# tungphambasement/DCNN

Hardware: AMD Instinct MI355X
Metric: images/sec (whole node) ResNet-18 Tiny-ImageNet training at 1/2/4/8 MI355X (higher is better)
Workload: dtype bf16; 1 GPU; model=resnet18_tiny_imagenet, global_batch=256, per_gpu_batch=256, parallelism=dp1, optimizer=adam, hipgraph=True, engine=native (C++ host API)

## Files before the change

### dcnn_amd/csrc/kernels/api.h

```cpp
#pragma once
#include <hip/hip_runtime.h>
#include <stdint.h>

#include "fusion_plan.h"
typedef __bf16 bf16;

namespace dcnn {
struct BnbArgs {
  const bf16* y; const bf16* x; const float* mean; const float* istd;
  const float* gamma; const float* beta; int mask_x;
};
struct NtArgs {
  const bf16* A; const bf16* B; void* C;
  int M, N, K; int lda, ldb, ldc; int mode;
  int nb, sh, sw, cs, gh, gw; int kh, kw, strh, strw, padh, padw;
  const float* bias; const bf16* residual; float* stats; int out_f32; int relu;
};
struct TnArgs {
  const bf16* dY; const bf16* X; float* slab; float* bias_slab;
  int M, N, P; int mode; int nb, sh, sw, cs, gh, gw; int kh, kw, strh, strw, padh, padw; int ldx; int k_per_split;
};
struct G2Args {
  const bf16* A; const bf16* B; bf16* C;
  unsigned a_bytes, b_bytes;
// ... 38 lines not shown
  int NB, H, W, Cs, N, ldb, ntaps;
  int tap_dy[9], tap_dx[9], tap_b[9];
  int TH, TW, IMG, HPR;
  const float* bias; const bf16* residual; float* stats; int relu;
  float* zero_ptr; int zero_n;
  BnbArgs bnb;
  float* Cf; const float* residual_f;
  int splits; float* part; unsigned* tickets;
};
void hconv(HConvArgs a, hipStream_t s);
int hconv_splits(int NB, int H, int W, int Cs, int N, int ntaps);
int hconv_tiles(int NB, int H, int W, int Cs, int N, int ntaps);
int hconv_tile_elems(int NB, int H, int W, int Cs, int N, int ntaps);
int hconv_split_target();
void gemm_t2_set_split_target(int t);
void hwgrad_set_split_target(int t);
void hconv3_set_max_splits(int n);
void g1s_set_waves_per_simd(int w);
void hconv_set_split_target(int t);
void hconv_set_split_min_work(int w);
void bn_set_vectorised(int on);
bool hconv_supported(int NB, int H, int W, int Cs, int N, int ntaps);
int hconv_stat_rows(int NB, int H, int W, int Cs, int N, int ntaps, int f32out);
bool hconv3_f32_try(const HConvArgs& a, hipStream_t s);
int hconv3_f32_splits(int NB, int H, int W, int Cs, int N, int ntaps);
bool hconv_v3(int NB, int H, int W, int Cs, int N, int ntaps);
void hconv3_enable(int on);
void hconv3_set_grid_cap(int n);
void hconv3_set_stamps(uintptr_t p);
struct HWArgs {
  const bf16* dY; const bf16* X; float* slab; float* bias_slab;
  unsigned dy_bytes, x_bytes;
  int NB, H, W, Cs, Co, ntaps;
  int tap_dy[9], tap_dx[9];
  int TH, TW, IMG, HPR, tiles_per_split;
  int ldy, ldx, npairs;
  int pair_yoff[3], pair_xoff[3], pair_bias[3];
};
void hwgrad(HWArgs a, int splits, hipStream_t s);
bool hwgrad_supported(int NB, int H, int W, int Cs, int Co, int ntaps);
int hwgrad_splits(int NB, int H, int W, int Cs, int Co);
bool hwgrad_f32_supported(int NB, int H, int W, int Cs, int Co);
int hwgrad_f32_splits(int NB, int H, int W, int Cs, int Co);
void hwgrad_f32(HWArgs a, int splits, hipStream_t s);
void hwgrad_set_version(int v);
bool hwgrad_s2_supported(int NB, int H, int W, int Cs, int Co);
int hwgrad_s2_splits(int NB, int H, int W, int Cs, int Co);
void hwgrad_s2(HWArgs a, int splits, hipStream_t s);

void gemm_nt(const NtArgs& a, hipStream_t s);
void gemm_g2(const G2Args& a, hipStream_t s);
void gemm_g2_set_splitk(int on);
int gemm_g2_splitk_enabled();
int gemm_g2_stat_rows(int M, int N);
int gemm_g2_row_tile(int M, int N);
void gemm_t2(T2Args a, int splits, hipStream_t s);
int g1s_rows(int M, int N, int K, int mode);
void g1s_enable(int on);
void g1s(const bf16* X, const bf16* Wt, bf16* Y, int M, int N, int K, int H, int W, int OH, int OW, int S,
         const float* bias, const bf16* residual, float* stats, int relu, float* zero_ptr, int zero_n, BnbArgs bnb,
         int mode, hipStream_t s);
int g1s_gen_rows(int M, int N, int Kc, int ntaps, int mode);
void g1s_gen(const bf16* X, const bf16* Wt, bf16* Y, int NB, int GH, int GW, int N, int Kc, int ldw,
             const std::vector<std::array<int, 3>>& taps, int H, int W, int OHo, int OWo, int OS, int ORY, int ORX,
             const bf16* residual, float* stats, float* zero_ptr, int zero_n, BnbArgs bnb, int mode, hipStream_t s);
int gemm_t2_splits(int M, int N, int P);
int gemm_nt_stat_rows(int M, int N);
void elementwise(int mode, int op, const float* a, const float* b, float* c, long n, float s0, float s1, hipStream_t s);
void reduce(int op, const float* a, const float* b, long n, float* workspace, float* out, hipStream_t s);
void fill_random(float* out, long n, uint64_t seed, float a, float b, int normal, hipStream_t s);
void transpose_batched(const float* in, float* out, int batch, int rows, int cols, hipStream_t s);
void transpose_batched16(const void* in, void* out, int batch, int rows, int cols, hipStream_t s);
void rows_copy(int kind, const void* src, int lds, void* dst, int ldd, long rows, int cols, hipStream_t s);
void nchw_cnhw(const float* in, float* out, int N, int C, int HW, int to_cnhw, hipStream_t s);
void pad_crop(const float* in, float* out, int NC, int H, int W, int OH, int OW, int top, int left, float value,
              hipStream_t s);
void gemm_g2f(const G2Args& a, hipStream_t s);
int gemm_g2f_stat_rows(int M, int N);
void gemm_t2f(T2Args a, int splits, hipStream_t s);
int gemm_t2f_splits(int M, int N, int P);
void set_f32_mode(int mode);
int get_f32_mode();
void conv_weight_transpose_f32(const float* w, float* wt, int Co, int T_, int Ci, hipStream_t s);
void gemm_tn(TnArgs a, int splits, hipStream_t s);
int gemm_tn_splits(int M, int N, int P);
int gemm_tn_k_per_split(int P, int splits);
int gemm_tn_bias_rows(int M);
struct ConvRouteGeom {
  int N, C, H, W, Co, KH, KW, SH, SW, PH, PW, OH, OW, g1s_mode;
};
enum ConvRoute : int { ROUTE_GENERIC = 0, ROUTE_GEMM_G2 = 1, ROUTE_HALO = 2, ROUTE_G1S = 3, ROUTE_HALO_S2 = 4 };
int conv_fwd_route(ConvRouteGeom g);
int conv_dgrad_route(ConvRouteGeom g);
int conv_wgrad_route(ConvRouteGeom g);
void splitk_reduce(const float* slab, float* out, long n, int splits, int accumulate, hipStream_t s);
void splitk_reduce2(const float* slab, float* out, long n, const float* bslab, float* bout, long nb, int splits,
                    int accumulate, hipStream_t s);

constexpr int kMaxRed = 48;
struct RedEnt { const float* slab; float* out; long n; int splits, unit0, chunks, groups, vec, wpc; };
struct MultiRed { int count; RedEnt e[kMaxRed]; };
void multi_splitk_reduce(MultiRed t, hipStream_t s);

int bn_partial_rows(long R, int C);
void bn_partial(int dtype, const void* x, const void* dy, const void* yout, void* dy_out, const float* mean,
                const float* istd, long R, int C, float* slab, int mode, float* zero_sums, hipStream_t s);
// ... 143 lines not shown
```

### dcnn_amd/csrc/kernels/bindings.cpp

```cpp
#include <tuple>
#include <pybind11/pybind11.h>
#include <pybind11/stl.h>
#include <algorithm>
#include <array>
#include <vector>
#include <hip/hip_runtime.h>
#include <stdint.h>

namespace py = pybind11;
#include "api.h"


using namespace dcnn;
void bind_runtime(py::module_& m);
void bind_rccl(py::module_& m);
template <typename T>
static inline T P(uintptr_t x) { return reinterpret_cast<T>(x); }
static inline hipStream_t S(uintptr_t x) { return reinterpret_cast<hipStream_t>(x); }

using Ptr4 = std::array<uintptr_t, 4>;
static BnbArgs bnb_of(const Ptr4& b) {
  return BnbArgs{P<const bf16*>(b[0]), P<const bf16*>(b[1]), P<const float*>(b[2]), P<const float*>(b[3])};
}

// ... 102 lines not shown
  m.def("hconv_stat_rows", &hconv_stat_rows);
  m.def("hconv_splits", &hconv_splits);
  m.def("hconv_tiles", &hconv_tiles);
  m.def("hconv_set_split_target", &hconv_set_split_target);
  m.def("hconv_set_split_min_work", &hconv_set_split_min_work);
  m.def("hconv_split_target", &hconv_split_target);
  m.def("gemm_t2_set_split_target", &gemm_t2_set_split_target);
  m.def("hwgrad_set_split_target", &hwgrad_set_split_target);
  m.def("hconv3_set_max_splits", &hconv3_set_max_splits);
  m.def("bn_set_vectorised", &bn_set_vectorised);
  m.def("hconv_tile_elems", &hconv_tile_elems);
  m.def("hconv3_set_grid_cap", &hconv3_set_grid_cap);
  m.def("hconv3_enable", &hconv3_enable);
  m.def("hconv_v3", &hconv_v3);
  m.def("hconv3_set_stamps", &hconv3_set_stamps);
  m.def("hwgrad",
        [](int kind, uintptr_t dY, uintptr_t X, uintptr_t slab, uintptr_t bias_slab, unsigned dy_bytes,
           unsigned x_bytes, int NB, int H, int W, int Cs, int Co, const WgradTaps& taps, int splits, int ldy, int ldx,
           const std::vector<std::array<int, 3>>& pairs, uintptr_t stream) {
          HWArgs a{};
          if (pairs.size() > 3) throw std::runtime_error("hwgrad: at most 3 operand pairs");
          a.npairs = (int)pairs.size(); a.ldy = ldy; a.ldx = ldx;
          for (size_t q = 0; q < pairs.size(); ++q) {
            a.pair_yoff[q] = pairs[q][0]; a.pair_xoff[q] = pairs[q][1]; a.pair_bias[q] = pairs[q][2];
          }
          a.dY = P<const bf16*>(dY); a.X = P<const bf16*>(X); a.slab = P<float*>(slab);
          a.bias_slab = P<float*>(bias_slab);
          a.dy_bytes = dy_bytes; a.x_bytes = x_bytes;
          a.NB = NB; a.H = H; a.W = W; a.Cs = Cs; a.Co = Co;
          if (kind == 1) {
            a.ntaps = 9;
            hwgrad_s2(a, splits, S(stream));
            return;
          }
          set_taps(a, taps, "hwgrad");
          if (kind == 2)
            hwgrad_f32(a, splits, S(stream));
          else
            hwgrad(a, splits, S(stream));
        });
  m.def("hwgrad_supported", &hwgrad_supported);
  m.def("hwgrad_s2_supported", &hwgrad_s2_supported);
  m.def("hwgrad_s2_splits", &hwgrad_s2_splits);
  m.def("hwgrad_f32_supported", &hwgrad_f32_supported);
  m.def("hwgrad_f32_splits", &hwgrad_f32_splits);
  m.def("split3_bf16", [](uintptr_t in, uintptr_t out, long rows, int C, int pattern, uintptr_t st) {
    split3_bf16(P<const float*>(in), P<bf16*>(out), rows, C, pattern, S(st));
  });
  m.def("hwgrad_splits", &hwgrad_splits);
  m.def("hwgrad_set_version", &hwgrad_set_version);
  m.def("gemm_g2f_stat_rows", &gemm_g2f_stat_rows);
  m.def("gemm_g2_set_splitk", &gemm_g2_set_splitk);
  m.def("gemm_g2_splitk_enabled", &gemm_g2_splitk_enabled);
  m.def("set_f32_mode", &set_f32_mode);
  m.def("get_f32_mode", &get_f32_mode);
  m.def("gemm_t2f_splits", &gemm_t2f_splits);
  m.def("conv_weight_transpose_f32", [](uintptr_t w, uintptr_t wt, int Co, int T_, int Ci, uintptr_t st) {
    conv_weight_transpose_f32(P<const float*>(w), P<float*>(wt), Co, T_, Ci, S(st));
  });
  m.def("gemm_g2", [](int f32, uintptr_t A, uintptr_t B, uintptr_t C, unsigned a_bytes, unsigned b_bytes, int M, int N,
                      int Cs, int H, int W, int GH, int GW, int SY, int SX, const ConvTaps& taps, int ldb, int ldc, int OH,
                      int OW, int OSY, int OSX, int ORY, int ORX, uintptr_t bias, uintptr_t residual, uintptr_t stats,
                      int relu, uintptr_t zero_ptr, int zero_n, Ptr4 bnb, uintptr_t stream,
                      const std::vector<std::array<int, 4>>& classes) {
    bind_gemm_g2(f32, A, B, C, a_bytes, b_bytes, M, N, Cs, H, W, GH, GW, SY, SX, taps, ldb, ldc, OH, OW, OSY, OSX, ORY, ORX,
                 bias, residual, stats, relu, zero_ptr, zero_n, bnb, stream, classes, -1);
  });
  m.def("gemm_g2_res_cls", &bind_gemm_g2);
  m.def("gemm_g2_plain", [](int f32, uintptr_t A, uintptr_t B, uintptr_t C, unsigned a_bytes, unsigned b_bytes, int M,
                            int N, int K, uintptr_t bias, uintptr_t residual, uintptr_t stats, int relu,
                            uintptr_t zero_ptr, int zero_n, uintptr_t stream) {
    bind_gemm_g2(f32, A, B, C, a_bytes, b_bytes, M, N, K, 1, 1, 1, 1, 1, 1, {{0, 0, 0, 0}}, K, N, 1, 1, 1, 1, 0, 0, bias,
                 residual, stats, relu, zero_ptr, zero_n, Ptr4{0, 0, 0, 0}, stream, {}, -1);
  });
  m.def("gemm_g2_stat_rows", &gemm_g2_stat_rows);
  for (auto [name, fn] : {std::pair<const char*, int (*)(ConvRouteGeom)>{"conv_fwd_route", &conv_fwd_route},
                          {"conv_dgrad_route", &conv_dgrad_route}, {"conv_wgrad_route", &conv_wgrad_route}})
    m.def(name, [fn](int N, int C, int H, int W, int Co, int KH, int KW, int SH, int SW, int PH, int PW, int OH, int OW,
                     int g1s_mode) { return fn(ConvRouteGeom{N, C, H, W, Co, KH, KW, SH, SW, PH, PW, OH, OW, g1s_mode}); });
  m.def("conv_fwd_taps", [](int C, int W, int KH, int KW, int PH, int PW) {
    ConvRouteGeom g{};
    g.W = W; g.KH = KH; g.KW = KW; g.PH = PH; g.PW = PW;
    return conv_fwd_taps(g, C);
  });
  m.def("conv_wgrad_taps", [](int KH, int KW, int PH, int PW) {
    ConvRouteGeom g{};
    g.KH = KH; g.KW = KW; g.PH = PH; g.PW = PW;
    return conv_wgrad_taps(g);
  });
  m.def("conv_dgrad_phases", [](int H, int W, int OW, int Co, int KH, int KW, int SH, int SW, int PH, int PW) {
    ConvRouteGeom g{};
    g.H = H; g.W = W; g.OW = OW; g.Co = Co; g.KH = KH; g.KW = KW; g.SH = SH; g.SW = SW; g.PH = PH; g.PW = PW;
    const DgradPhases p = conv_dgrad_phases(g);
    std::vector<std::array<int, 6>> ph;
    for (const DgradPhase& c : p.phases) ph.push_back({c.ry, c.rx, c.GH, c.GW, c.t0, c.nt});
    return std::make_pair(ph, p.taps);
  });
  m.attr("ROUTE_GENERIC") = (int)ROUTE_GENERIC;
  m.attr("ROUTE_GEMM_G2") = (int)ROUTE_GEMM_G2;
  m.attr("ROUTE_HALO") = (int)ROUTE_HALO;
  m.attr("ROUTE_G1S") = (int)ROUTE_G1S;
  m.attr("ROUTE_HALO_S2") = (int)ROUTE_HALO_S2;
  m.def("plan_sequence_fusions", &plan_sequence_fusions);
  m.def("plan_residual_fusions", &plan_residual_fusions, py::arg("main_kinds"), py::arg("short_kinds"),
        py::arg("act_ok"), py::arg("act_identity") = false);
  for (auto [name, v] : {std::pair<const char*, int>{"FK_OTHER", FK_OTHER}, {"FK_CONV", FK_CONV}, {"FK_BN", FK_BN},
// ... 455 lines not shown
```

### dcnn_amd/csrc/kernels/gemm2.hip

```cpp
#include <cstdio>
#include <cstdlib>
#include <map>
#include <mutex>
#include <vector>

#include "common.h"
#include "api.h"

namespace dcnn {

typedef __attribute__((address_space(3))) void lds_void;

__device__ __forceinline__ int xcd_remap2(int bid, int nwg) {
  const int xcd = bid & 7, q = nwg >> 3, r = nwg & 7;
  const int base = xcd < r ? xcd * (q + 1) : r * (q + 1) + (xcd - r) * q;
  return base + (bid >> 3);
}

__device__ __forceinline__ void glds16(__amdgpu_buffer_rsrc_t rsrc, char* lds, unsigned voff) {
  __builtin_amdgcn_raw_ptr_buffer_load_lds(rsrc, (lds_void*)lds, 16, voff, 0, 0, 0);
}

constexpr unsigned kOOB = 0x80000000u;

__device__ __forceinline__ unsigned g2_div(int n, const unsigned* f) {
  return fdiv((unsigned)n, FastDiv{f[0], f[1], f[2]});
}

template <int BM, int BN, int BK, bool UNI, int NST>
struct G2 {
  static constexpr int CPR = BK / 8;
  static constexpr int RPI = 64 / CPR;
  static constexpr int RPB = 256 / (BK * 2);
  static constexpr int A_INS = BM / RPI / 4;
  static constexpr int B_INS = BN / RPI / 4;
  static constexpr int TM = BM / 32, TN = BN / 32;
  static constexpr int STAGE = (BM + BN) * BK * 2;
  static constexpr int EPI_PITCH = BN * 2 + 16;
  static constexpr int LDS = (NST * STAGE > BM * EPI_PITCH) ? NST * STAGE : BM * EPI_PITCH;
  static constexpr int INS = A_INS + B_INS;
  __device__ static __forceinline__ int swz(int row) { return (row / RPB) % CPR; }
  __device__ static __forceinline__ int off(int row, int ch) { return row * (BK * 2) + ((ch ^ swz(row)) << 4); }
};

template <int BM, int BN, int EPI_PITCH>
__device__ __forceinline__ void g2_epilogue2(const G2Args& p, char* smem, int m0, int n0, int tm, int cls, int mcls,
                                             int ory, int orx) {
  const int tid = threadIdx.x;
  constexpr int CG = BN / 8;
  constexpr int RSTEP = 256 / CG;
  const int cg = tid % CG, r0 = tid / CG;
  const int ncol = n0 + cg * 8;
  const bool col_ok = ncol < p.N;
  float s[8], q[8], mu[8], is[8], pv[8];
#pragma unroll
  for (int v = 0; v < 8; ++v) s[v] = q[v] = mu[v] = is[v] = pv[v] = 0.f;
  const bool bnb = p.bnb.x != nullptr;
  if (bnb && col_ok) {
#pragma unroll
    for (int v = 0; v < 8; ++v) { mu[v] = p.bnb.mean[ncol + v]; is[v] = p.bnb.istd[ncol + v]; }
  }
  float piv_col = 0.f;
  if (p.stats && !bnb) {
    unpack8(*reinterpret_cast<const uint4*>(smem + cg * 16), pv);
    if (tid < BN) piv_col = (float)*reinterpret_cast<const bf16*>(smem + tid * 2);
  }
  const int ghw = p.GH * p.GW;
  auto orow_of = [&](int row) {
    const int ml = m0 + row - mcls;
    const int img = (int)g2_div(ml, p.fd_ghw), rem = ml - img * ghw;
    const int gy = (int)g2_div(rem, p.fd_gw), gx = rem - gy * p.GW;
    return ((long)img * p.OH + gy * p.OSY + ory) * p.OW + gx * p.OSX + orx;
  };
  const bool has_res = p.residual != nullptr, has_y = bnb && p.bnb.y != nullptr, has_x = bnb && p.stats;
  const bool res_compact = p.res_cls >= 0;
  const bool load_res = has_res && (!res_compact || cls == p.res_cls);
  constexpr int NR = BM / RSTEP;
  uint4 c_res[NR], c_y[NR], c_x[NR];
#pragma unroll
  for (int i = 0; i < NR; ++i) {
    c_res[i] = c_y[i] = c_x[i] = uint4{0u, 0u, 0u, 0u};
    const int row = r0 + i * RSTEP;
    if (m0 + row >= p.M || !col_ok) continue;
    const long o = orow_of(row) * p.ldc + ncol;
    if (load_res)
      c_res[i] = *reinterpret_cast<const uint4*>(p.residual + (res_compact ? (long)(m0 + row - mcls) * p.ldc + ncol : o));
    if (has_y) c_y[i] = *reinterpret_cast<const uint4*>(p.bnb.y + o);
    if (has_x) c_x[i] = *reinterpret_cast<const uint4*>(p.bnb.x + o);
  }
#pragma unroll
  for (int i = 0; i < NR; ++i) {
    const int row = r0 + i * RSTEP;
    const int m = m0 + row;
    if (m < p.M && col_ok) {
      const long orow = orow_of(row);
// ... 9 lines not shown
#pragma unroll
        for (int v = 0; v < 8; ++v) f[v] = fmaxf(f[v], 0.f);
      }
      if (has_y) {
        float yo[8];
        unpack8(c_y[i], yo);
#pragma unroll
        for (int v = 0; v < 8; ++v) f[v] = yo[v] > 0.f ? f[v] : 0.f;
      }
      const uint4 o = pack8(f);
      *reinterpret_cast<uint4*>(reinterpret_cast<bf16*>(p.C) + orow * p.ldc + ncol) = o;
      if (p.stats) {
        float g[8];
        unpack8(o, g);
        if (bnb) {
          float xv[8];
          unpack8(c_x[i], xv);
#pragma unroll
          for (int v = 0; v < 8; ++v) { s[v] += g[v]; q[v] += g[v] * (xv[v] - mu[v]) * is[v]; }
        } else {
#pragma unroll
          for (int v = 0; v < 8; ++v) { const float d = g[v] - pv[v]; s[v] += d; q[v] += d * d; }
        }
      }
    }
  }
  if (p.stats) {
    __syncthreads();
    float* red = reinterpret_cast<float*>(smem);
#pragma unroll
    for (int v = 0; v < 8; ++v) {
      red[(r0 * 2 + 0) * BN + cg * 8 + v] = s[v];
      red[(r0 * 2 + 1) * BN + cg * 8 + v] = q[v];
    }
    __syncthreads();
    if (bnb) {
      for (int c = tid; c < 2 * BN; c += 256) {
        const int which = c / BN, cc = c % BN;
        if (n0 + cc < p.N) {
          float a = 0.f;
          for (int k = 0; k < RSTEP; ++k) a += red[(k * 2 + which) * BN + cc];
          p.stats[((long)tm * 2 + which) * p.N + n0 + cc] = a;
        }
      }
    } else if (tid < BN && n0 + tid < p.N) {
      float a = 0.f, b = 0.f;
      for (int k = 0; k < RSTEP; ++k) { a += red[(k * 2 + 0) * BN + tid]; b += red[(k * 2 + 1) * BN + tid]; }
      const float cnt = (float)min(BM, p.M - m0);
      store_welford(p.stats, tm, p.N, n0 + tid, welford_from_shifted(cnt, piv_col, a, b));
    }
  }
}

template <int BM, int BN, int BK, bool UNI, int NST, bool SPLIT = false>
__global__ void __launch_bounds__(256, 2) gemm_g2_kernel(G2Args p) {
  prefetch_kernargs<sizeof(G2Args)>();
  using T = G2<BM, BN, BK, UNI, NST>;
  __shared__ __attribute__((aligned(16))) char smem[T::LDS];
  const int tid = threadIdx.x, lane = tid & 63, wid = tid >> 6;
  const int wm = wid >> 1, wn = wid & 1;
  const int tiles_n = (p.N + BN - 1) / BN;
  const int lt_all = xcd_remap2(blockIdx.x, gridDim.x);
  const int ks = SPLIT ? p.ksplit : 1;
  const int lt = SPLIT ? lt_all / ks : lt_all, kslice = SPLIT ? lt_all - lt * ks : 0;
  const int tm = lt / tiles_n, tn = lt % tiles_n;
  const int cls = p.ncls > 1 ? tm % p.ncls : 0;
  const int m0 = p.ncls > 1 ? cls * p.cls_rows + (tm / p.ncls) * BM : tm * BM, n0 = tn * BN;
  const int mcls = cls * p.cls_rows;
  const int ct0 = p.cls_t0[cls], ntp = p.cls_nt[cls];
  const int ory = p.cls_ory[cls], orx = p.cls_orx[cls];

  const __amdgpu_buffer_rsrc_t rsA = __builtin_amdgcn_make_buffer_rsrc((void*)p.A, (short)0, p.a_bytes, 0x00020000);
  const __amdgpu_buffer_rsrc_t rsB = __builtin_amdgcn_make_buffer_rsrc((void*)p.B, (short)0, p.b_bytes, 0x00020000);
  if (p.zero_ptr && blockIdx.x == 0) {
    for (int i = tid; i < p.zero_n; i += 256) p.zero_ptr[i] = 0.f;
    asm volatile("s_waitcnt vmcnt(0)" ::: "memory");
  }

  const int ch = lane % T::CPR;
  unsigned a_base[T::A_INS];
  uint64_t a_mask[T::A_INS];
  int a_lch[T::A_INS];
#pragma unroll
  for (int i = 0; i < T::A_INS; ++i) {
    const int row = (wid * T::A_INS + i) * T::RPI + lane / T::CPR;
    a_lch[i] = ch ^ T::swz(row);
    const int m = m0 + row;
    uint64_t mask = 0;
    unsigned base = 0;
    if (m < p.M) {
      const int ml = m - mcls;
      const int img = (int)g2_div(ml, p.fd_ghw), rem = ml - img * p.GH * p.GW;
      const int gy = (int)g2_div(rem, p.fd_gw), gx = rem - gy * p.GW;
      const int y0 = gy * p.SY, x0 = gx * p.SX;
      base = (unsigned)((((long)img * p.H + y0) * p.W + x0) * p.Cs * 2);
      for (int t = 0; t < ntp; ++t) {
        const int sy = y0 + p.tap_dy[ct0 + t], sx = x0 + p.tap_dx[ct0 + t];
        if (sy >= 0 && sy < p.H && sx >= 0 && sx < p.W) mask |= (1ull << t);
      }
    }
    a_base[i] = base;
    a_mask[i] = mask;
  }
  unsigned b_base[T::B_INS];
  bool b_ok[T::B_INS];
  int b_lch[T::B_INS];
#pragma unroll
  for (int i = 0; i < T::B_INS; ++i) {
    const int row = (wid * T::B_INS + i) * T::RPI + lane / T::CPR;
    b_lch[i] = ch ^ T::swz(row);
    const int n = n0 + row;
    b_ok[i] = n < p.N;
    b_base[i] = (unsigned)((long)n * p.ldb * 2);
  }

  const int tab_src = lane < ntp ? p.tap_srcoff[ct0 + lane] : 0;
  const int tab_b = lane < ntp ? p.tap_b[ct0 + lane] : 0;
  int st_t = 0, st_c = 0;

  auto stage = [&](int buf, int k0) {
    char* As = smem + buf * T::STAGE;
    char* Bs = As + BM * BK * 2;
    if constexpr (UNI) {
      const int t = st_t, c0 = st_c;
      st_c += BK;
      if (st_c >= p.Cs) { st_c -= p.Cs; ++st_t; }
      const bool tok = t < ntp;
      const int tl = tok ? t : 0;
      const int src = __builtin_amdgcn_readlane(tab_src, tl), tb = __builtin_amdgcn_readlane(tab_b, tl);
#pragma unroll
      for (int i = 0; i < T::A_INS; ++i) {
        const int c = c0 + a_lch[i] * 8;
        const bool ok = tok && c < p.Cs && ((a_mask[i] >> tl) & 1ull);
        const unsigned voff = ok ? a_base[i] + (unsigned)(src * 2 + c * 2) : kOOB;
        glds16(rsA, As + (wid * T::A_INS + i) * 1024, voff);
      }
#pragma unroll
      for (int i = 0; i < T::B_INS; ++i) {
        const int c = c0 + b_lch[i] * 8;
        const bool ok = b_ok[i] && tok && c < p.Cs;
        const unsigned voff = ok ? b_base[i] + (unsigned)((tb + c) * 2) : kOOB;
        glds16(rsB, Bs + (wid * T::B_INS + i) * 1024, voff);
      }
      return;
    }
#pragma unroll
    for (int i = 0; i < T::A_INS; ++i) {
      const int k = k0 + a_lch[i] * 8;
      const int t = k / p.Cs, c = k - t * p.Cs;
      const bool ok = t < ntp && c < p.Cs && ((a_mask[i] >> t) & 1ull);
      const unsigned voff = ok ? a_base[i] + (unsigned)(p.tap_srcoff[ct0 + t] * 2 + c * 2) : kOOB;
      glds16(rsA, As + (wid * T::A_INS + i) * 1024, voff);
    }
#pragma unroll
    for (int i = 0; i < T::B_INS; ++i) {
      const int k = k0 + b_lch[i] * 8;
      const int t = k / p.Cs, c = k - t * p.Cs;
      const bool ok = b_ok[i] && t < ntp && c < p.Cs;
      const unsigned voff = ok ? b_base[i] + (unsigned)((p.tap_b[ct0 + t] + c) * 2) : kOOB;
      glds16(rsB, Bs + (wid * T::B_INS + i) * 1024, voff);
    }
  };

  f32x4 acc[T::TM][T::TN];
#pragma unroll
  for (int i = 0; i < T::TM; ++i)
#pragma unroll
    for (int j = 0; j < T::TN; ++j) acc[i][j] = f32x4{0.f, 0.f, 0.f, 0.f};

  const int K = ntp * p.Cs;
  const int nk_all = (K + BK - 1) / BK;
  const int kb = SPLIT ? (int)((long)nk_all * kslice / ks) : 0;
  const int nk = SPLIT ? (int)((long)nk_all * (kslice + 1) / ks) - kb : nk_all;
  if constexpr (UNI && SPLIT) {
    const int k0 = kb * BK;
    st_t = k0 / p.Cs;
    st_c = k0 - st_t * p.Cs;
  }
  auto compute = [&](int buf) {
    const char* As = smem + buf * T::STAGE;
    const char* Bs = As + BM * BK * 2;
    constexpr int KK = BK / 32;
    bf16x8 a[KK][T::TM], b[KK][T::TN];
#pragma unroll
    for (int kk = 0; kk < KK; ++kk) {
      const int c = kk * 4 + (lane >> 4);
#pragma unroll
      for (int i = 0; i < T::TM; ++i)
        a[kk][i] = *reinterpret_cast<const bf16x8*>(As + T::off(wm * (BM / 2) + i * 16 + (lane & 15), c));
#pragma unroll
      for (int j = 0; j < T::TN; ++j)
        b[kk][j] = *reinterpret_cast<const bf16x8*>(Bs + T::off(wn * (BN / 2) + j * 16 + (lane & 15), c));
    }
#pragma unroll
    for (int kk = 0; kk < KK; ++kk) {
      __builtin_amdgcn_s_setprio(1);
#pragma unroll
      for (int i = 0; i < T::TM; ++i)
#pragma unroll
        for (int j = 0; j < T::TN; ++j)
          acc[i][j] = __builtin_amdgcn_mfma_f32_16x16x32_bf16(a[kk][i], b[kk][j], acc[i][j], 0, 0, 0);
      __builtin_amdgcn_s_setprio(0);
    }
  };
  const int kofs = kb * BK;
  if constexpr (NST == 2) {
    stage(0, kofs);
    asm volatile("s_waitcnt vmcnt(0)" ::: "memory");
    __syncthreads();
    int cur = 0;
    for (int kt = 0; kt < nk; ++kt) {
      if (kt + 1 < nk) stage(cur ^ 1, kofs + (kt + 1) * BK);
      compute(cur);
      asm volatile("s_waitcnt vmcnt(0)" ::: "memory");
      __syncthreads();
      cur ^= 1;
    }
  } else {
    stage(0, kofs);
    if (nk > 1) {
      stage(1, kofs + BK);
      asm volatile("s_waitcnt vmcnt(%0)" ::"n"(T::INS) : "memory");
    } else {
      asm volatile("s_waitcnt vmcnt(0)" ::: "memory");
    }
    __builtin_amdgcn_s_barrier();
    int cur = 0;
    for (int kt = 0; kt < nk; ++kt) {
      const bool more = kt + 2 < nk;
      if (more) stage(cur == 0 ? 2 : cur - 1, kofs + (kt + 2) * BK);
      compute(cur);
      if (more) asm volatile("s_waitcnt vmcnt(%0) lgkmcnt(0)" ::"n"(T::INS) : "memory");
      else asm volatile("s_waitcnt vmcnt(0) lgkmcnt(0)" ::: "memory");
      __builtin_amdgcn_s_barrier();
      asm volatile("" ::: "memory");
      cur = cur == 2 ? 0 : cur + 1;
    }
  }

  if constexpr (SPLIT) {
    float* out = p.kpart + (long)kslice * p.M * p.N;
#pragma unroll
    for (int i = 0; i < T::TM; ++i)
#pragma unroll
      for (int j = 0; j < T::TN; ++j) {
        const int n = n0 + wn * (BN / 2) + j * 16 + (lane & 15);
#pragma unroll
        for (int r = 0; r < 4; ++r) {
          const int m = m0 + wm * (BM / 2) + i * 16 + (lane >> 4) * 4 + r;
          if (m < p.M && n < p.N) out[(long)m * p.N + n] = acc[i][j][r];
        }
      }
    return;
  }
#pragma unroll
  for (int j = 0; j < T::TN; ++j) {
    const int col = wn * (BN / 2) + j * 16 + (lane & 15);
    const float bv = (p.bias && n0 + col < p.N) ? p.bias[n0 + col] : 0.f;
#pragma unroll
    for (int i = 0; i < T::TM; ++i)
#pragma unroll
      for (int r = 0; r < 4; ++r) {
        const int row = wm * (BM / 2) + i * 16 + (lane >> 4) * 4 + r;
        *reinterpret_cast<bf16*>(smem + row * T::EPI_PITCH + col * 2) = (bf16)(acc[i][j][r] + bv);
      }
  }
  __syncthreads();
  g2_epilogue2<BM, BN, T::EPI_PITCH>(p, smem, m0, n0, tm, cls, mcls, ory, orx);
}

constexpr int kG2MaxSplit = 8;

template <int BM, int BN>
__global__ void __launch_bounds__(256, 2) g2_splitk_epi_kernel(G2Args p) {
  prefetch_kernargs<sizeof(G2Args)>();
  constexpr int EPI_PITCH = BN * 2 + 16;
  constexpr int RSTEP = 256 / (BN / 8);
  constexpr int L1 = BM * EPI_PITCH, L2 = RSTEP * 2 * BN * 4;
  constexpr int LDS = L1 > L2 ? L1 : L2;
  __shared__ __attribute__((aligned(16))) char smem[LDS];
  const int tid = threadIdx.x;
  const int tiles_n = (p.N + BN - 1) / BN;
  const int lt = xcd_remap2(blockIdx.x, gridDim.x);
  const int tm = lt / tiles_n, tn = lt % tiles_n;
  const int m0 = tm * BM, n0 = tn * BN;
  constexpr int C4 = BN / 4, RS = 256 / C4;
  const int c4 = tid % C4, rr = tid / C4;
  const int n = n0 + c4 * 4;
  float bv[4] = {0.f, 0.f, 0.f, 0.f};
  if (p.bias && n < p.N) {
#pragma unroll
    for (int v = 0; v < 4; ++v) bv[v] = p.bias[n + v];
  }
  const long slice = (long)p.M * p.N;
  const int ks = p.ksplit;
  static_assert((BM / RS) % 2 == 0, "row pairs");
#pragma unroll 1
  for (int row = rr; row < BM; row += 2 * RS) {
    float4 v[2][kG2MaxSplit];
#pragma unroll
    for (int h = 0; h < 2; ++h) {
      const int m = m0 + row + h * RS;
      const bool ok = m < p.M && n < p.N;
      const float* src = p.kpart + (long)(ok ? m : 0) * p.N + (ok ? n : 0);
#pragma unroll
// ... 217 lines not shown
    __syncthreads();
    red[tid] = bias_acc;
    __syncthreads();
    if (tid < BM) {
      float s = 0.f;
      for (int k = 0; k < RS; ++k) s += red[tid + k * BM];
      if (m0 + tid < p.M) p.bias_slab[(long)split * p.M + m0 + tid] = s;
    }
  }
}

static int g2_stages() {
  static const int v = [] {
    const char* e = std::getenv("DCNN_G2_STAGES");
    return e ? std::atoi(e) : 0;
  }();
  return v == 2 || v == 3 ? v : 0;
}

static float* g2_kpart(size_t bytes, hipStream_t s) {
  static std::mutex mu;
  static std::map<std::pair<int, hipStream_t>, std::pair<float*, size_t>> ws;
  static std::vector<float*> retired;
  int dev = 0;
  DCNN_HIP_CHECK(hipGetDevice(&dev));
  std::lock_guard<std::mutex> g(mu);
  auto& e = ws[{dev, s}];
  if (e.second < bytes) {
    hipStreamCaptureStatus st = hipStreamCaptureStatusNone;
    DCNN_HIP_CHECK(hipStreamIsCapturing(s, &st));
    if (st != hipStreamCaptureStatusNone) {
      const std::pair<float*, size_t>* best = nullptr;
      for (const auto& kv : ws)
        if (kv.first.first == dev && kv.second.second >= bytes && (!best || kv.second.second > best->second))
          best = &kv.second;
      if (best) return best->first;
      throw std::runtime_error("gemm_g2: split-K workspace must grow outside graph capture (run a step eagerly first)");
    }
    if (e.first) retired.push_back(e.first);
    const size_t n = bytes > (size_t)(32 << 20) ? bytes : (size_t)(32 << 20);
    DCNN_HIP_CHECK(hipMalloc(&e.first, n));
    e.second = n;
  }
  return e.first;
}

static int g_g2_splitk = [] {
  const char* v = std::getenv("DCNN_G2_SPLITK");
  return (v && v[0] == '0') ? 0 : 1;
}();
void gemm_g2_set_splitk(int on) { g_g2_splitk = on; }
int gemm_g2_splitk_enabled() { return g_g2_splitk; }

static int g2_ksplit(const G2Args& a, int tiles, int bk) {
  if (g_g2_splitk != 1 || a.ntaps != 1 || a.ncls > 1 || a.Cs < 1024 || tiles >= 256) return 1;
  if (a.tap_dy[0] != 0 || a.tap_dx[0] != 0 || a.SY != 1 || a.SX != 1 || a.OSY != 1 || a.OSX != 1 ||
      a.GH != a.H || a.GW != a.W || a.OH != a.GH || a.OW != a.GW || a.ldc != a.N)
    return 1;
  const int nk = (a.Cs + bk - 1) / bk;
  int ks = (512 + tiles - 1) / tiles;
  if (ks > nk / 4) ks = nk / 4;
  if (ks > kG2MaxSplit) ks = kG2MaxSplit;
  return ks < 2 ? 1 : ks;
}

template <int BM, int BN, int BK, bool UNI>
static void launch_g2(const G2Args& a0, hipStream_t s) {
  const int tiles = ((a0.M + BM - 1) / BM) * ((a0.N + BN - 1) / BN);
  G2Args a = a0;
  a.ksplit = 1;
  if constexpr (BK == 64 && UNI) {
    a.ksplit = g2_ksplit(a0, tiles, BK);
    if (a.ksplit > 1) {
      a.kpart = g2_kpart((size_t)a.ksplit * a.M * a.N * 4, s);
      hipLaunchKernelGGL((gemm_g2_kernel<BM, BN, BK, UNI, 2, true>), dim3(tiles * a.ksplit), dim3(256), 0, s, a);
      DCNN_LAUNCH_CHECK();
      a.zero_ptr = nullptr;
      hipLaunchKernelGGL((g2_splitk_epi_kernel<BM, BN>), dim3(tiles), dim3(256), 0, s, a);
      DCNN_LAUNCH_CHECK();
      return;
    }
  }
  int ksteps = 0;
  for (int c = 0; c < a.ncls; ++c) {
    const int k = a.cls_nt[c] * ((a.Cs + BK - 1) / BK);
    ksteps = k > ksteps ? k : ksteps;
  }
  constexpr bool deep = !(BM == 128 && BN == 64);
  const int stages = g2_stages() ? g2_stages()
                                 : ((deep && 2 * G2<BM, BN, BK, UNI, 3>::LDS <= 163840 && ksteps > 1) ? 3 : 2);
  if (stages == 3)
    hipLaunchKernelGGL((gemm_g2_kernel<BM, BN, BK, UNI, 3>), dim3(tiles), dim3(256), 0, s, a);
  else
    hipLaunchKernelGGL((gemm_g2_kernel<BM, BN, BK, UNI, 2>), dim3(tiles), dim3(256), 0, s, a);
  DCNN_LAUNCH_CHECK();
}

void g2_tile(int M, int N, int* bm, int* bn) {
  static const int force = [] {
    const char* e = std::getenv("DCNN_G2_TILE");
    int m = 0, n = 0;
    return (e && std::sscanf(e, "%dx%d", &m, &n) == 2) ? m * 1000 + n : 0;
  }();
  if (force) { *bm = force / 1000; *bn = force % 1000; return; }
  auto tiles = [&](int m, int n) { return (long)((M + m - 1) / m) * ((N + n - 1) / n); };
  if (g_g2_splitk == 2 && N <= 256 && tiles(64, 64) < 192) { *bm = 32; *bn = 64; return; }
  if (N >= 128 && tiles(128, 128) >= 480) { *bm = 128; *bn = 128; return; }
  if (N >= 128 && tiles(64, 128) >= 480 && tiles(128, 64) < 640) { *bm = 64; *bn = 128; return; }
  if (tiles(128, 64) >= 480 || N < 128) {
    *bm = tiles(128, 64) >= 400 ? 128 : 64;
    *bn = 64;
    return;
  }
  if (tiles(64, 128) >= 400) { *bm = 64; *bn = 128; return; }
  *bm = 64;
  *bn = 64;
}

int gemm_g2_stat_rows(int M, int N) {
  int bm, bn;
  g2_tile(M, N, &bm, &bn);
  return (M + bm - 1) / bm;
}

int gemm_g2_row_tile(int M, int N) {
  int bm, bn;
  g2_tile(M, N, &bm, &bn);
  return bm;
}

void gemm_g2(const G2Args& a_in, hipStream_t s) {
  G2Args a = a_in;
  if (a.N % 8 != 0 || a.Cs % 8 != 0 || a.ldb % 8 != 0 || a.ldc % 8 != 0 || a.ntaps > 64 || a.ntaps < 1)
    throw std::runtime_error("gemm_g2: unsupported shape (needs N, Cs, ldb, ldc multiples of 8, 1..64 taps)");
  int bm, bn;
  g2_tile(a.M, a.N, &bm, &bn);
  if (a.ncls <= 1) {
    a.ncls = 1; a.cls_rows = a.M;
    a.cls_t0[0] = 0; a.cls_nt[0] = a.ntaps; a.cls_ory[0] = a.ORY; a.cls_orx[0] = a.ORX;
  } else {
    if (a.ncls > 4 || a.cls_rows <= 0 || a.cls_rows % bm || a.ncls * a.cls_rows != a.M)
      throw std::runtime_error("gemm_g2: grouped classes need <= 4 classes of equal rows, a multiple of the row tile");
    for (int c = 0; c < a.ncls; ++c)
      if (a.cls_nt[c] < 0 || a.cls_t0[c] < 0 || a.cls_t0[c] + a.cls_nt[c] > a.ntaps)
        throw std::runtime_error("gemm_g2: class tap range out of bounds");
  }
  if (a.res_cls >= 0) {
// ... 84 lines not shown
```

Baseline: 94610 images/sec.

## Add opt-in register-resident GEMM epilogue and issue B tile before A-row setup

Adds an alternative epilogue for the implicit-GEMM conv kernel that works directly on the accumulator registers. It swaps the MFMA operand order and remaps the A rows and B columns so each lane holds 8 contiguous output channels. It then applies bias, residual, ReLU, the BN-backward mask and the per-tile statistics reduction without first staging the output tile through shared memory. The new path is off unless DCNN_G2_REG_EPI=1 is set. Separately, on every path the prologue now issues the first B-tile load before computing the A-row tap masks, and builds those masks from readlane'd tap offsets, so the global loads overlap the index setup. The trade-off is more template instances and higher register pressure in the opt-in variant.

```diff
diff --git a/dcnn_amd/csrc/kernels/api.h b/dcnn_amd/csrc/kernels/api.h
--- a/dcnn_amd/csrc/kernels/api.h
+++ b/dcnn_amd/csrc/kernels/api.h
@@ -114,6 +114,9 @@
 void gemm_g2(const G2Args& a, hipStream_t s);
 void gemm_g2_set_splitk(int on);
 int gemm_g2_splitk_enabled();
+void gemm_g2_set_reg_epilogue(int on);
+int gemm_g2_reg_epilogue_enabled();
+int gemm_g2_last_epilogue();
 int gemm_g2_stat_rows(int M, int N);
 int gemm_g2_row_tile(int M, int N);
 void gemm_t2(T2Args a, int splits, hipStream_t s);
diff --git a/dcnn_amd/csrc/kernels/bindings.cpp b/dcnn_amd/csrc/kernels/bindings.cpp
--- a/dcnn_amd/csrc/kernels/bindings.cpp
+++ b/dcnn_amd/csrc/kernels/bindings.cpp
@@ -178,6 +178,9 @@
   m.def("gemm_g2f_stat_rows", &gemm_g2f_stat_rows);
   m.def("gemm_g2_set_splitk", &gemm_g2_set_splitk);
   m.def("gemm_g2_splitk_enabled", &gemm_g2_splitk_enabled);
+  m.def("gemm_g2_set_reg_epilogue", &gemm_g2_set_reg_epilogue);
+  m.def("gemm_g2_reg_epilogue_enabled", &gemm_g2_reg_epilogue_enabled);
+  m.def("gemm_g2_last_epilogue", &gemm_g2_last_epilogue);
   m.def("set_f32_mode", &set_f32_mode);
   m.def("get_f32_mode", &get_f32_mode);
   m.def("gemm_t2f_splits", &gemm_t2f_splits);
diff --git a/dcnn_amd/csrc/kernels/gemm2.hip b/dcnn_amd/csrc/kernels/gemm2.hip
--- a/dcnn_amd/csrc/kernels/gemm2.hip
+++ b/dcnn_amd/csrc/kernels/gemm2.hip
@@ -41,6 +41,15 @@
   static constexpr int INS = A_INS + B_INS;
   __device__ static __forceinline__ int swz(int row) { return (row / RPB) % CPR; }
   __device__ static __forceinline__ int off(int row, int ch) { return row * (BK * 2) + ((ch ^ swz(row)) << 4); }
+  static constexpr int RSTEP = 256 / (BN / 8);
+  static constexpr int RED = RSTEP * 2 * BN * 4;
+  static constexpr int LDS_PIV = (NST * STAGE > RED + BN * 2) ? NST * STAGE : RED + BN * 2;
+  __device__ static __forceinline__ int reg_arow(int wm, int i, int l16) {
+    return RSTEP == 32 ? i * 32 + wm * 16 + l16 : (wm * TM + i) * 16 + l16;
+  }
+  __device__ static __forceinline__ int reg_bcol(int wn, int j, int l16) {
+    return wn * (BN / 2) + (j >> 1) * 32 + (l16 >> 2) * 8 + ((l16 >> 1) & 1) * 4 + (j & 1) * 2 + (l16 & 1);
+  }
 };
 
 template <int BM, int BN, int EPI_PITCH>
@@ -156,11 +165,182 @@
   }
 }
 
-template <int BM, int BN, int BK, bool UNI, int NST, bool SPLIT = false>
+template <int BM, int BN, int BK, bool UNI, int NST, int EPI>
+__device__ __forceinline__ void g2_epilogue_reg(const G2Args& p, char* smem, f32x4 (&acc)[BM / 32][BN / 32], int m0,
+                                                int n0, int tm, int cls, int mcls, int ory, int orx) {
+  using T = G2<BM, BN, BK, UNI, NST>;
+  constexpr int TM = T::TM, NG = T::TN / 2, RSTEP = T::RSTEP;
+  constexpr bool BNB = EPI >= 2, HAS_Y = EPI == 3;
+  constexpr int GPB = TM * NG > 4 ? 1 : NG;
+  const int tid = threadIdx.x, lane = tid & 63, wid = tid >> 6;
+  const int wm = wid >> 1, wn = wid & 1, l16 = lane & 15, q = lane >> 4;
+  int ncol[NG];
+  bool col_ok[NG];
+  float bv[NG][8];
+#pragma unroll
+  for (int g = 0; g < NG; ++g) {
+    ncol[g] = n0 + wn * (BN / 2) + g * 32 + q * 8;
+    col_ok[g] = ncol[g] < p.N;
+#pragma unroll
+    for (int v = 0; v < 8; ++v) bv[g][v] = (p.bias && col_ok[g]) ? p.bias[ncol[g] + v] : 0.f;
+  }
+  const int ghw = p.GH * p.GW;
+  bool rok[TM];
+  int ml[TM];
+  long orow[TM];
+#pragma unroll
+  for (int i = 0; i < TM; ++i) {
+    const int row = T::reg_arow(wm, i, l16);
+    rok[i] = m0 + row < p.M;
+    ml[i] = m0 + row - mcls;
+    orow[i] = 0;
+    if (rok[i]) {
+      const int img = (int)g2_div(ml[i], p.fd_ghw), rem = ml[i] - img * ghw;
+      const int gy = (int)g2_div(rem, p.fd_gw), gx = rem - gy * p.GW;
+      orow[i] = (((long)img * p.OH + gy * p.OSY + ory) * p.OW + gx * p.OSX + orx) * p.ldc;
+    }
+  }
+  const bool has_res = p.residual != nullptr, has_x = BNB && p.stats;
+  const bool res_compact = p.res_cls >= 0;
+  const bool load_res = has_res && (!res_compact || cls == p.res_cls);
+  uint4 o[TM][NG], c_x[TM][NG];
+  char* piv = smem + T::RED;
+#pragma unroll
+  for (int g0 = 0; g0 < NG; g0 += GPB) {
+    uint4 c_res[TM][GPB], c_y[TM][GPB];
+#pragma unroll
+    for (int i = 0; i < TM; ++i)
+#pragma unroll
+      for (int gg = 0; gg < GPB; ++gg) {
+        const int g = g0 + gg;
+        c_res[i][gg] = c_y[i][gg] = c_x[i][g] = o[i][g] = uint4{0u, 0u, 0u, 0u};
+        if (!rok[i] || !col_ok[g]) continue;
+        const long off = orow[i] + ncol[g];
+        if (load_res)
+          c_res[i][gg] = *reinterpret_cast<const uint4*>(p.residual + (res_compact ? (long)ml[i] * p.ldc + ncol[g] : off));
+        if constexpr (HAS_Y) c_y[i][gg] = *reinterpret_cast<const uint4*>(p.bnb.y + off);
+        if constexpr (BNB) {
+          if (has_x) c_x[i][g] = *reinterpret_cast<const uint4*>(p.bnb.x + off);
+        }
+      }
+#pragma unroll
+    for (int i = 0; i < TM; ++i)
+#pragma unroll
+      for (int gg = 0; gg < GPB; ++gg) {
+        const int g = g0 + gg;
+        if (!rok[i] || !col_ok[g]) continue;
+        float f[8];
+#pragma unroll
+        for (int v = 0; v < 8; ++v) f[v] = acc[i][2 * g + ((v >> 1) & 1)][(v >> 2) * 2 + (v & 1)] + bv[g][v];
+        const uint4 staged = pack8(f);
+        if constexpr (EPI == 1) {
+          if (i == 0 && wm == 0 && l16 == 0) *reinterpret_cast<uint4*>(piv + (ncol[g] - n0) * 2) = staged;
+        }
+        unpack8(staged, f);
+        if (has_res) {
+          float rr[8];
+          unpack8(c_res[i][gg], rr);
+#pragma unroll
+          for (int v = 0; v < 8; ++v) f[v] += rr[v];
+        }
+        if (p.relu) {
+#pragma unroll
+          for (int v = 0; v < 8; ++v) f[v] = fmaxf(f[v], 0.f);
+        }
+        if constexpr (HAS_Y) {
+          float yo[8];
+          unpack8(c_y[i][gg], yo);
+#pragma unroll
+          for (int v = 0; v < 8; ++v) f[v] = yo[v] > 0.f ? f[v] : 0.f;
+        }
+        o[i][g] = pack8(f);
+        *reinterpret_cast<uint4*>(reinterpret_cast<bf16*>(p.C) + orow[i] + ncol[g]) = o[i][g];
+      }
+  }
+  if constexpr (EPI >= 1) {
+    if (!p.stats) return;
+    float* red = reinterpret_cast<float*>(smem);
+    constexpr int NSEG = RSTEP == 32 ? 1 : 2;
+    const int k = RSTEP == 32 ? wm * 16 + l16 : l16, seg = RSTEP == 32 ? 0 : wm;
+    float pv[NG][8], mu[NG][8], is[NG][8];
+    float piv_col = 0.f;
+    if constexpr (EPI == 1) {
+      __syncthreads();
+#pragma unroll
+      for (int g = 0; g < NG; ++g) unpack8(*reinterpret_cast<const uint4*>(piv + (ncol[g] - n0) * 2), pv[g]);
+      if (tid < BN) piv_col = (float)*reinterpret_cast<const bf16*>(piv + tid * 2);
+    } else {
+#pragma unroll
+      for (int g = 0; g < NG; ++g)
+#pragma unroll
+        for (int v = 0; v < 8; ++v) {
+          mu[g][v] = col_ok[g] ? p.bnb.mean[ncol[g] + v] : 0.f;
+          is[g][v] = col_ok[g] ? p.bnb.istd[ncol[g] + v] : 0.f;
+        }
+    }
+#pragma unroll
+    for (int sg = 0; sg < NSEG; ++sg) {
+      if (sg == seg) {
+#pragma unroll
+        for (int g = 0; g < NG; ++g) {
+          const int cb = wn * (BN / 2) + g * 32 + q * 8;
+          float s[8], qq[8];
+#pragma unroll
+          for (int v = 0; v < 8; ++v) {
+            s[v] = sg ? red[(k * 2 + 0) * BN + cb + v] : 0.f;
+            qq[v] = sg ? red[(k * 2 + 1) * BN + cb + v] : 0.f;
+          }
+#pragma unroll
+          for (int i = 0; i < TM; ++i) {
+            if (!rok[i] || !col_ok[g]) continue;
+            float gv[8];
+            unpack8(o[i][g], gv);
+            if constexpr (BNB) {
+              float xv[8];
+              unpack8(c_x[i][g], xv);
+#pragma unroll
+              for (int v = 0; v < 8; ++v) { s[v] += gv[v]; qq[v] += gv[v] * (xv[v] - mu[g][v]) * is[g][v]; }
+            } else {
+#pragma unroll
+              for (int v = 0; v < 8; ++v) { const float d = gv[v] - pv[g][v]; s[v] += d; qq[v] += d * d; }
+            }
+          }
+#pragma unroll
+          for (int v = 0; v < 8; ++v) {
+            red[(k * 2 + 0) * BN + cb + v] = s[v];
+            red[(k * 2 + 1) * BN + cb + v] = qq[v];
+          }
+        }
+      }
+      __syncthreads();
+    }
+    if constexpr (BNB) {
+      for (int c = tid; c < 2 * BN; c += 256) {
+        const int which = c / BN, cc = c % BN;
+        if (n0 + cc < p.N) {
+          float a = 0.f;
+          for (int kk = 0; kk < RSTEP; ++kk) a += red[(kk * 2 + which) * BN + cc];
+          p.stats[((long)tm * 2 + which) * p.N + n0 + cc] = a;
+        }
+      }
+    } else if (tid < BN && n0 + tid < p.N) {
+      float a = 0.f, b = 0.f;
+      for (int kk = 0; kk < RSTEP; ++kk) { a += red[(kk * 2 + 0) * BN + tid]; b += red[(kk * 2 + 1) * BN + tid]; }
+      const float cnt = (float)min(BM, p.M - m0);
+      store_welford(p.stats, tm, p.N, n0 + tid, welford_from_shifted(cnt, piv_col, a, b));
+    }
+  }
+}
+
+
+template <int BM, int BN, int BK, bool UNI, int NST, bool SPLIT = false, int EPI = -1>
 __global__ void __launch_bounds__(256, 2) gemm_g2_kernel(G2Args p) {
   prefetch_kernargs<sizeof(G2Args)>();
   using T = G2<BM, BN, BK, UNI, NST>;
-  __shared__ __attribute__((aligned(16))) char smem[T::LDS];
+  constexpr bool REG = EPI >= 0;
+  static_assert(!(SPLIT && REG), "the split-K instance leaves the epilogue to g2_splitk_epi_kernel");
+  static_assert(NST * T::STAGE >= T::RED, "the statistics reduce buffer lives in the stage ring");
+  __shared__ __attribute__((aligned(16))) char smem[EPI == 1 ? T::LDS_PIV : (REG ? NST * T::STAGE : T::LDS)];
   const int tid = threadIdx.x, lane = tid & 63, wid = tid >> 6;
   const int wm = wid >> 1, wn = wid & 1;
   const int tiles_n = (p.N + BN - 1) / BN;
@@ -185,27 +365,6 @@
   unsigned a_base[T::A_INS];
   uint64_t a_mask[T::A_INS];
   int a_lch[T::A_INS];
-#pragma unroll
-  for (int i = 0; i < T::A_INS; ++i) {
-    const int row = (wid * T::A_INS + i) * T::RPI + lane / T::CPR;
-    a_lch[i] = ch ^ T::swz(row);
-    const int m = m0 + row;
-    uint64_t mask = 0;
-    unsigned base = 0;
-    if (m < p.M) {
-      const int ml = m - mcls;
-      const int img = (int)g2_div(ml, p.fd_ghw), rem = ml - img * p.GH * p.GW;
-      const int gy = (int)g2_div(rem, p.fd_gw), gx = rem - gy * p.GW;
-      const int y0 = gy * p.SY, x0 = gx * p.SX;
-      base = (unsigned)((((long)img * p.H + y0) * p.W + x0) * p.Cs * 2);
-      for (int t = 0; t < ntp; ++t) {
-        const int sy = y0 + p.tap_dy[ct0 + t], sx = x0 + p.tap_dx[ct0 + t];
-        if (sy >= 0 && sy < p.H && sx >= 0 && sx < p.W) mask |= (1ull << t);
-      }
-    }
-    a_base[i] = base;
-    a_mask[i] = mask;
-  }
   unsigned b_base[T::B_INS];
   bool b_ok[T::B_INS];
   int b_lch[T::B_INS];
@@ -220,58 +379,9 @@
 
   const int tab_src = lane < ntp ? p.tap_srcoff[ct0 + lane] : 0;
   const int tab_b = lane < ntp ? p.tap_b[ct0 + lane] : 0;
+  const int tab_dy = lane < ntp ? p.tap_dy[ct0 + lane] : 0;
+  const int tab_dx = lane < ntp ? p.tap_dx[ct0 + lane] : 0;
   int st_t = 0, st_c = 0;
-
-  auto stage = [&](int buf, int k0) {
-    char* As = smem + buf * T::STAGE;
-    char* Bs = As + BM * BK * 2;
-    if constexpr (UNI) {
-      const int t = st_t, c0 = st_c;
-      st_c += BK;
-      if (st_c >= p.Cs) { st_c -= p.Cs; ++st_t; }
-      const bool tok = t < ntp;
-      const int tl = tok ? t : 0;
-      const int src = __builtin_amdgcn_readlane(tab_src, tl), tb = __builtin_amdgcn_readlane(tab_b, tl);
-#pragma unroll
-      for (int i = 0; i < T::A_INS; ++i) {
-        const int c = c0 + a_lch[i] * 8;
-        const bool ok = tok && c < p.Cs && ((a_mask[i] >> tl) & 1ull);
-        const unsigned voff = ok ? a_base[i] + (unsigned)(src * 2 + c * 2) : kOOB;
-        glds16(rsA, As + (wid * T::A_INS + i) * 1024, voff);
-      }
-#pragma unroll
-      for (int i = 0; i < T::B_INS; ++i) {
-        const int c = c0 + b_lch[i] * 8;
-        const bool ok = b_ok[i] && tok && c < p.Cs;
-        const unsigned voff = ok ? b_base[i] + (unsigned)((tb + c) * 2) : kOOB;
-        glds16(rsB, Bs + (wid * T::B_INS + i) * 1024, voff);
-      }
-      return;
-    }
-#pragma unroll
-    for (int i = 0; i < T::A_INS; ++i) {
-      const int k = k0 + a_lch[i] * 8;
-      const int t = k / p.Cs, c = k - t * p.Cs;
-      const bool ok = t < ntp && c < p.Cs && ((a_mask[i] >> t) & 1ull);
-      const unsigned voff = ok ? a_base[i] + (unsigned)(p.tap_srcoff[ct0 + t] * 2 + c * 2) : kOOB;
-      glds16(rsA, As + (wid * T::A_INS + i) * 1024, voff);
-    }
-#pragma unroll
-    for (int i = 0; i < T::B_INS; ++i) {
-      const int k = k0 + b_lch[i] * 8;
-      const int t = k / p.Cs, c = k - t * p.Cs;
-      const bool ok = b_ok[i] && t < ntp && c < p.Cs;
-      const unsigned voff = ok ? b_base[i] + (unsigned)((p.tap_b[ct0 + t] + c) * 2) : kOOB;
-      glds16(rsB, Bs + (wid * T::B_INS + i) * 1024, voff);
-    }
-  };
-
-  f32x4 acc[T::TM][T::TN];
-#pragma unroll
-  for (int i = 0; i < T::TM; ++i)
-#pragma unroll
-    for (int j = 0; j < T::TN; ++j) acc[i][j] = f32x4{0.f, 0.f, 0.f, 0.f};
-
   const int K = ntp * p.Cs;
   const int nk_all = (K + BK - 1) / BK;
   const int kb = SPLIT ? (int)((long)nk_all * kslice / ks) : 0;
@@ -281,6 +391,91 @@
     st_t = k0 / p.Cs;
     st_c = k0 - st_t * p.Cs;
   }
+
+  auto stage = [&](int buf, int k0, bool do_a = true, bool do_b = true) {
+    char* As = smem + buf * T::STAGE;
+    char* Bs = As + BM * BK * 2;
+    if constexpr (UNI) {
+      const int t = st_t, c0 = st_c;
+      if (do_a) {
+        st_c += BK;
+        if (st_c >= p.Cs) { st_c -= p.Cs; ++st_t; }
+      }
+      const bool tok = t < ntp;
+      const int tl = tok ? t : 0;
+      const int src = do_a ? __builtin_amdgcn_readlane(tab_src, tl) : 0;
+      const int tb = do_a ? __builtin_amdgcn_readlane(tab_b, tl) : p.tap_b[ct0 + tl];
+#pragma unroll
+      for (int i = 0; do_a && i < T::A_INS; ++i) {
+        const int c = c0 + a_lch[i] * 8;
+        const bool ok = tok && c < p.Cs && ((a_mask[i] >> tl) & 1ull);
+        const unsigned voff = ok ? a_base[i] + (unsigned)(src * 2 + c * 2) : kOOB;
+        glds16(rsA, As + (wid * T::A_INS + i) * 1024, voff);
+      }
+#pragma unroll
+      for (int i = 0; do_b && i < T::B_INS; ++i) {
+        const int c = c0 + b_lch[i] * 8;
+        const bool ok = b_ok[i] && tok && c < p.Cs;
+        const unsigned voff = ok ? b_base[i] + (unsigned)((tb + c) * 2) : kOOB;
+        glds16(rsB, Bs + (wid * T::B_INS + i) * 1024, voff);
+      }
+      return;
+    }
+#pragma unroll
+    for (int i = 0; do_a && i < T::A_INS; ++i) {
+      const int k = k0 + a_lch[i] * 8;
+      const int t = k / p.Cs, c = k - t * p.Cs;
+      const bool ok = t < ntp && c < p.Cs && ((a_mask[i] >> t) & 1ull);
+      const unsigned voff = ok ? a_base[i] + (unsigned)(p.tap_srcoff[ct0 + t] * 2 + c * 2) : kOOB;
+      glds16(rsA, As + (wid * T::A_INS + i) * 1024, voff);
+    }
+#pragma unroll
+    for (int i = 0; do_b && i < T::B_INS; ++i) {
+      const int k = k0 + b_lch[i] * 8;
+      const int t = k / p.Cs, c = k - t * p.Cs;
+      const bool ok = b_ok[i] && t < ntp && c < p.Cs;
+      const unsigned voff = ok ? b_base[i] + (unsigned)((p.tap_b[ct0 + t] + c) * 2) : kOOB;
+      glds16(rsB, Bs + (wid * T::B_INS + i) * 1024, voff);
+    }
+  };
+
+  const int kofs = kb * BK;
+  stage(0, kofs, false, true);
+
+  {
+    int y0[T::A_INS], x0[T::A_INS];
+    bool mok[T::A_INS];
+#pragma unroll
+    for (int i = 0; i < T::A_INS; ++i) {
+      const int row = (wid * T::A_INS + i) * T::RPI + lane / T::CPR;
+      a_lch[i] = ch ^ T::swz(row);
+      const int m = m0 + row;
+      mok[i] = m < p.M;
+      const int ml = mok[i] ? m - mcls : 0;
+      const int img = (int)g2_div(ml, p.fd_ghw), rem = ml - img * p.GH * p.GW;
+      const int gy = (int)g2_div(rem, p.fd_gw), gx = rem - gy * p.GW;
+      y0[i] = gy * p.SY;
+      x0[i] = gx * p.SX;
+      a_base[i] = mok[i] ? (unsigned)((((long)img * p.H + y0[i]) * p.W + x0[i]) * p.Cs * 2) : 0u;
+      a_mask[i] = 0;
+    }
+    for (int t = 0; t < ntp; ++t) {
+      const int dy = __builtin_amdgcn_readlane(tab_dy, t), dx = __builtin_amdgcn_readlane(tab_dx, t);
+      const uint64_t bit = 1ull << t;
+#pragma unroll
+      for (int i = 0; i < T::A_INS; ++i) {
+        const int sy = y0[i] + dy, sx = x0[i] + dx;
+        if (mok[i] && (unsigned)sy < (unsigned)p.H && (unsigned)sx < (unsigned)p.W) a_mask[i] |= bit;
+      }
+    }
+  }
+
+  f32x4 acc[T::TM][T::TN];
+#pragma unroll
+  for (int i = 0; i < T::TM; ++i)
+#pragma unroll
+    for (int j = 0; j < T::TN; ++j) acc[i][j] = f32x4{0.f, 0.f, 0.f, 0.f};
+
   auto compute = [&](int buf) {
     const char* As = smem + buf * T::STAGE;
     const char* Bs = As + BM * BK * 2;
@@ -290,11 +485,15 @@
     for (int kk = 0; kk < KK; ++kk) {
       const int c = kk * 4 + (lane >> 4);
 #pragma unroll
-      for (int i = 0; i < T::TM; ++i)
-        a[kk][i] = *reinterpret_cast<const bf16x8*>(As + T::off(wm * (BM / 2) + i * 16 + (lane & 15), c));
-#pragma unroll
-      for (int j = 0; j < T::TN; ++j)
-        b[kk][j] = *reinterpret_cast<const bf16x8*>(Bs + T::off(wn * (BN / 2) + j * 16 + (lane & 15), c));
+      for (int i = 0; i < T::TM; ++i) {
+        const int row = REG ? T::reg_arow(wm, i, lane & 15) : wm * (BM / 2) + i * 16 + (lane & 15);
+        a[kk][i] = *reinterpret_cast<const bf16x8*>(As + T::off(row, c));
+      }
+#pragma unroll
+      for (int j = 0; j < T::TN; ++j) {
+        const int col = REG ? T::reg_bcol(wn, j, lane & 15) : wn * (BN / 2) + j * 16 + (lane & 15);
+        b[kk][j] = *reinterpret_cast<const bf16x8*>(Bs + T::off(col, c));
+      }
     }
 #pragma unroll
     for (int kk = 0; kk < KK; ++kk) {
@@ -302,14 +501,15 @@
 #pragma unroll
       for (int i = 0; i < T::TM; ++i)
 #pragma unroll
-        for (int j = 0; j < T::TN; ++j)
-          acc[i][j] = __builtin_amdgcn_mfma_f32_16x16x32_bf16(a[kk][i], b[kk][j], acc[i][j], 0, 0, 0);
+        for (int j = 0; j < T::TN; ++j) {
+          if constexpr (REG) acc[i][j] = __builtin_amdgcn_mfma_f32_16x16x32_bf16(b[kk][j], a[kk][i], acc[i][j], 0, 0, 0);
+          else acc[i][j] = __builtin_amdgcn_mfma_f32_16x16x32_bf16(a[kk][i], b[kk][j], acc[i][j], 0, 0, 0);
+        }
       __builtin_amdgcn_s_setprio(0);
     }
   };
-  const int kofs = kb * BK;
   if constexpr (NST == 2) {
-    stage(0, kofs);
+    stage(0, kofs, true, false);
     asm volatile("s_waitcnt vmcnt(0)" ::: "memory");
     __syncthreads();
     int cur = 0;
@@ -321,7 +521,7 @@
       cur ^= 1;
     }
   } else {
-    stage(0, kofs);
+    stage(0, kofs, true, false);
     if (nk > 1) {
       stage(1, kofs + BK);
       asm volatile("s_waitcnt vmcnt(%0)" ::"n"(T::INS) : "memory");
@@ -355,6 +555,10 @@
           if (m < p.M && n < p.N) out[(long)m * p.N + n] = acc[i][j][r];
         }
       }
+    return;
+  }
+  if constexpr (REG) {
+    g2_epilogue_reg<BM, BN, BK, UNI, NST, EPI>(p, smem, acc, m0, n0, tm, cls, mcls, ory, orx);
     return;
   }
 #pragma unroll
@@ -678,6 +882,15 @@
 void gemm_g2_set_splitk(int on) { g_g2_splitk = on; }
 int gemm_g2_splitk_enabled() { return g_g2_splitk; }
 
+static int g_g2_reg_epi = [] {
+  const char* v = std::getenv("DCNN_G2_REG_EPI");
+  return (v && v[0] == '1') ? 1 : 0;
+}();
+static int g_g2_last_epi = -1;
+void gemm_g2_set_reg_epilogue(int on) { g_g2_reg_epi = on ? 1 : 0; }
+int gemm_g2_reg_epilogue_enabled() { return g_g2_reg_epi; }
+int gemm_g2_last_epilogue() { return g_g2_last_epi; }
+
 static int g2_ksplit(const G2Args& a, int tiles, int bk) {
   if (g_g2_splitk != 1 || a.ntaps != 1 || a.ncls > 1 || a.Cs < 1024 || tiles >= 256) return 1;
   if (a.tap_dy[0] != 0 || a.tap_dx[0] != 0 || a.SY != 1 || a.SX != 1 || a.OSY != 1 || a.OSX != 1 ||
@@ -688,6 +901,20 @@
   if (ks > nk / 4) ks = nk / 4;
   if (ks > kG2MaxSplit) ks = kG2MaxSplit;
   return ks < 2 ? 1 : ks;
+}
+
+template <int BM, int BN, int BK, bool UNI, int NST>
+static void launch_g2_epi(const G2Args& a, int tiles, hipStream_t s) {
+#define DCNN_G2_EPI(E) \
+  hipLaunchKernelGGL((gemm_g2_kernel<BM, BN, BK, UNI, NST, false, E>), dim3(tiles), dim3(256), 0, s, a)
+  const bool bnb = a.bnb.x != nullptr;
+  if (!g_g2_reg_epi) DCNN_G2_EPI(-1);
+  else if (bnb && a.bnb.y) DCNN_G2_EPI(3);
+  else if (bnb) DCNN_G2_EPI(2);
+  else if (a.stats) DCNN_G2_EPI(1);
+  else DCNN_G2_EPI(0);
+#undef DCNN_G2_EPI
+  g_g2_last_epi = g_g2_reg_epi;
 }
 
 template <int BM, int BN, int BK, bool UNI>
@@ -704,6 +931,7 @@
       a.zero_ptr = nullptr;
       hipLaunchKernelGGL((g2_splitk_epi_kernel<BM, BN>), dim3(tiles), dim3(256), 0, s, a);
       DCNN_LAUNCH_CHECK();
+      g_g2_last_epi = 0;
       return;
     }
   }
@@ -716,9 +944,9 @@
   const int stages = g2_stages() ? g2_stages()
                                  : ((deep && 2 * G2<BM, BN, BK, UNI, 3>::LDS <= 163840 && ksteps > 1) ? 3 : 2);
   if (stages == 3)
-    hipLaunchKernelGGL((gemm_g2_kernel<BM, BN, BK, UNI, 3>), dim3(tiles), dim3(256), 0, s, a);
+    launch_g2_epi<BM, BN, BK, UNI, 3>(a, tiles, s);
   else
-    hipLaunchKernelGGL((gemm_g2_kernel<BM, BN, BK, UNI, 2>), dim3(tiles), dim3(256), 0, s, a);
+    launch_g2_epi<BM, BN, BK, UNI, 2>(a, tiles, s);
   DCNN_LAUNCH_CHECK();
 }
 
```

Result: no change. 95090 images/sec (median of 6 runs) (+0.5%).
